# dremovd/PPO

Measured on AMD Instinct MI355X. Metric: env-steps/sec (Pong-shaped synthetic, 256 envs/GPU), higher is better.
Workload: dtype f32

## Files before the change

ppo_amd/csrc/stack_fused.hip:

```cpp
#include <cstdlib>
#include <type_traits>

#include "common.h"
#include "conv_stage.h"
#include "mfma.h"

#ifndef PPO_TAIL_SPLIT
#define PPO_TAIL_SPLIT 2
#endif

namespace ppo {
namespace {

constexpr int kScrPitchS = 20;

struct StackTailArgs {
    const float *in;
    const float *w[4];
    const float *bias[4];
    const float *mask[4];
    float *save[4];
    int n_images;
};

// ... 141 lines not shown
                    if (s < KS) {
#pragma unroll
                        for (int m = 0; m < MT; ++m)
#pragma unroll
                            for (int n = 0; n < NT; ++n) acc[n][m] = mfma16(wa[n][s], bv[u][m], acc[n][m]);
                    }
                }
                __builtin_amdgcn_sched_barrier(0);
            }

            __builtin_amdgcn_sched_barrier(0);
            load_weights((layer + 1) & 3);
            float *dst = smem + (odd ? 0 : S::LDS_MAP);
            float *save = a.save[layer];
            __builtin_amdgcn_sched_barrier(0);
            float skip[MT][NT][4];
#pragma unroll
            for (int m = 0; m < MT; ++m)
#pragma unroll
                for (int n = 0; n < NT; ++n)
#pragma unroll
                    for (int r = 0; r < 4; ++r)
                        skip[m][n][r] = odd ? smem[((n0 + n) * 16 + g * 4 + r) * PLANE + G + W + (pix[m] < S::NPIX ? pix[m] : 0)] : 0.f;
#pragma unroll
            for (int m = 0; m < MT; ++m) {
                if (pix[m] < S::NPIX) {
#pragma unroll
                    for (int n = 0; n < NT; ++n)
#pragma unroll
                        for (int r = 0; r < 4; ++r) {
                            const int co = (n0 + n) * 16 + g * 4 + r;
                            const int lo = co * PLANE + G + W + pix[m];
                            float val = acc[n][m][r] + bias_r[n][r];
                            if constexpr (BACKWARD) val = gate[m][n][r] > 0.f ? val : 0.f;
                            if (odd) val = val + skip[m][n][r];
                            dst[lo] = val;
                            if (save) save[img_off + (size_t)co * (H * W) + pix[m]] = val;
                        }
                }
            }
        }
    }
}

template <int C, int H, int W, int MT, int NW, int NSPLIT, bool BACKWARD>
int launch_stack_tail(const StackTailArgs &args, hipStream_t st)
{
    using S = StackCfg<C, H, W, MT, NW, NSPLIT>;
    constexpr auto kern = stack_tail_kernel<C, H, W, MT, NW, NSPLIT, BACKWARD>;
    int nb = 0;
    if (int rc = prepare_kernel<kern>("stack_tail", S::LDS_BYTES, S::WAVES * 64, &nb)) return rc;
    const int wg_per_cu = nb < 1 ? 1 : nb;
    int grid = 256 * wg_per_cu;
    if (grid > args.n_images) grid = args.n_images;
    hipLaunchKernelGGL(kern, dim3(grid), dim3(S::WAVES * 64), S::LDS_BYTES, st, args);
    return check_launch("stack_tail_kernel");
}

template <int C, int H, int W, int TR>
struct ShiftCfg {
    static_assert(C == 16, "one channel tile per wave");
    static constexpr int NW = 16;
    static constexpr int GW = 8;
    static constexpr int G = 4;
    static constexpr int PITCH = W + 2;
    static constexpr int ROWS = H + 6;
    static constexpr int PLANE_RAW = ROWS * PITCH + 2 * G;
    static constexpr int PLANE = PLANE_RAW + ((16 - PLANE_RAW % 32) + 32) % 32;
    static constexpr int KS = 9 * (C / 4);
    static constexpr int NBANDS = (H + TR - 1) / TR;
    static constexpr int NPIX = TR * W;
    static constexpr int MTILES = (NPIX + 15) / 16;
    static constexpr int MT = MTILES / GW;
    static constexpr int LDS_MAP = C * PLANE;
    static constexpr int SCR = MT * 16 * kScrPitchS;
    static constexpr size_t LDS_BYTES = (size_t)(LDS_MAP + GW * SCR) * 4;
    static_assert(H % TR == 0 && MTILES == MT * GW, "whole bands, tiles split evenly over a group's waves");
    static_assert((H * W) % 4 == 0 && NPIX % 4 == 0 && W % 2 == 0, "float4 epilogue on whole quads");
    static_assert(LDS_BYTES <= 160 * 1024, "map + scratch must fit the CU's LDS");
};

template <int C, int H, int W, int TR, bool BACKWARD>
__global__ __launch_bounds__(1024) void stack_shift_kernel(StackTailArgs a)
{
    using S = ShiftCfg<C, H, W, TR>;
    constexpr int KS = S::KS, PLANE = S::PLANE, PITCH = S::PITCH, G = S::G, MT = S::MT, NW = S::NW;
    extern __shared__ __align__(16) float smem[];
    const int tid = threadIdx.x, lane = tid & 63, l15 = lane & 15, g = lane >> 4, wave = tid >> 6;
    const int grp = __builtin_amdgcn_readfirstlane(wave / S::GW), wv = wave % S::GW;
    const int ch = lane >> 2, quad = lane & 3;
    float *scr = smem + S::LDS_MAP + wv * S::SCR;

    zero_lds<S::LDS_MAP, NW * 64>(smem, tid);

    int lofs[MT], p4[MT], po[MT][2];
#pragma unroll
    for (int m = 0; m < MT; ++m) {
        const int p = (wv * MT + m) * 16 + l15;
        lofs[m] = G + (p / W) * PITCH + p % W - 1 + g * PLANE;
        p4[m] = (wv * MT + m) * 16 + quad * 4;
        po[m][0] = (p4[m] / W) * PITCH + p4[m] % W;
        po[m][1] = ((p4[m] + 2) / W) * PITCH + (p4[m] + 2) % W;
    }

    for (int img = blockIdx.x; img < a.n_images; img += gridDim.x) {
        const size_t img_off = (size_t)img * C * H * W;
        __syncthreads();
        for (int i = tid; i < C * 6 * W; i += NW * 64) {
            const int c = i / (6 * W), r = (i / W) % 6, x = i % W;
            smem[c * PLANE + G + (r < 5 ? r : H + 5) * PITCH + x] = 0.f;
        }
        {
            constexpr int W2 = W / 2, RP = 64 / W2, NQ = H / RP;
            static_assert(H % RP == 0, "whole requests");
            const int w0 = __builtin_amdgcn_readfirstlane(wave);
            const bool live = lane < RP * W2;
            const int ls = live ? lane : RP * W2 - 1;
            for (int c = w0; c < C; c += NW) {
                const float2 *g2 = reinterpret_cast<const float2 *>(a.in + img_off + (size_t)c * H * W) + ls;
                float *l0 = smem + c * PLANE + G + (5 + ls / W2) * PITCH + (ls % W2) * 2;
                float2 v[NQ];
#pragma unroll
                for (int q = 0; q < NQ; ++q) v[q] = g2[q * RP * W2];
#pragma unroll
                for (int q = 0; q < NQ; ++q) {
                    const float2 o = BACKWARD ? v[q] : make_float2(relu1(v[q].x), relu1(v[q].y));
                    if (live) *reinterpret_cast<float2 *>(l0 + q * RP * PITCH) = o;
                }
            }
        }

#pragma unroll 1
        for (int layer = 0; layer < 4; ++layer) {
            float wa[KS];
            const float4 *pw = reinterpret_cast<const float4 *>(a.w[layer]);
#pragma unroll
            for (int s4 = 0; s4 < KS / 4; ++s4) {
                const float4 v = pw[s4 * 64 + lane];
                wa[4 * s4 + 0] = v.x, wa[4 * s4 + 1] = v.y, wa[4 * s4 + 2] = v.z, wa[4 * s4 + 3] = v.w;
            }
            const float bias_c = BACKWARD ? 0.f : a.bias[layer][ch];
            const int odd = layer & 1;
            const float *res = odd ? (layer == 1 ? a.in : a.save[1]) + img_off : nullptr;
            const float *mask = BACKWARD ? a.mask[layer] + img_off : nullptr;
            float *save = a.save[layer] ? a.save[layer] + img_off : nullptr;
            const __amdgpu_buffer_rsrc_t mask_b = buffer_of(mask, mask != nullptr), res_b = buffer_of(res, res != nullptr);
            const int in_row = 5 - layer;

            f32x4 acc[MT];
            float4 gate4[MT], res4[MT];

            __syncthreads();
#pragma unroll 1
            for (int hs = 0; hs <= S::NBANDS; ++hs) {
                if ((hs & 1) == grp) {
                    if (hs < S::NBANDS) {
                        const int y0 = hs * TR;
                        const int chan_off = ch * (H * W) + y0 * W;
#pragma unroll
                        for (int m = 0; m < MT; ++m) {
                            const bool live = p4[m] < S::NPIX;
                            const int off = live ? (chan_off + p4[m]) * 4 : kOutside;
                            if constexpr (BACKWARD) gate4[m] = buffer_f32x4(mask_b, off);
                            res4[m] = buffer_f32x4(res_b, off);
                        }
                        constexpr int CS_HI = ((C / 4 - 1) * 4 * PLANE + 2 * PITCH + 2) * 4 > 65535 ? C / 8 : C / 4;
                        static_assert(((C / 4 - 1 - (CS_HI < C / 4 ? CS_HI : 0)) * 4 * PLANE + 2 * PITCH + 2) * 4 <= 65535 &&
                                      ((CS_HI - 1) * 4 * PLANE + 2 * PITCH + 2) * 4 <= 65535, "operand offsets fit the instruction");
                        using lds_cvf = const volatile __attribute__((address_space(3))) float;
                        lds_cvf *vsmem = (lds_cvf *)smem;
                        int base[MT], base_hi[MT];
#pragma unroll
                        for (int m = 0; m < MT; ++m) {
                            base[m] = lofs[m] + (y0 - 1 + in_row) * PITCH;
                            base_hi[m] = base[m] + CS_HI * 4 * PLANE;
                            if constexpr (CS_HI < C / 4) asm volatile("" : "+v"(base_hi[m]));
                            acc[m] = f32x4{0.f, 0.f, 0.f, 0.f};
                        }
                        constexpr int SB = 2;
                        constexpr int NB = (KS + SB - 1) / SB;
                        float raw[2][SB][MT];
                        auto load_block = [&](int j, float (&r)[SB][MT]) {
#pragma unroll
                            for (int u = 0; u < SB; ++u) {
                                const int s = j * SB + u;
                                if (s < KS) {
                                    const int tap = s / (C / 4), cs = s % (C / 4);
                                    const int tap_off = (tap / 3) * PITCH + (tap % 3);
#pragma unroll
                                    for (int m = 0; m < MT; ++m)
                                        r[u][m] = cs < CS_HI ? vsmem[base[m] + cs * 4 * PLANE + tap_off]
                                                             : vsmem[base_hi[m] + (cs - CS_HI) * 4 * PLANE + tap_off];
                                }
                            }
                        };
                        load_block(0, raw[0]);
#pragma unroll
                        for (int j = 0; j < NB; ++j) {
                            __builtin_amdgcn_sched_barrier(0);
                            if (j + 1 < NB) load_block(j + 1, raw[(j + 1) & 1]);
                            __builtin_amdgcn_sched_barrier(0);
#pragma unroll
                            for (int u = 0; u < SB; ++u) {
                                const int s = j * SB + u;
                                if (s < KS) {
#pragma unroll
                                    for (int m = 0; m < MT; ++m) acc[m] = mfma16(wa[s], raw[j & 1][u][m], acc[m]);
                                }
                            }
                            __builtin_amdgcn_sched_barrier(0);
                        }
                    } else if (layer < 3) {
                        for (int i = tid % (S::GW * 64); i < C * W; i += S::GW * 64)
                            smem[(i / W) * PLANE + G + (H + in_row - 1) * PITCH + i % W] = 0.f;
                    }
                } else if (hs >= 1) {
                    const int y0 = (hs - 1) * TR;
                    const int chan_off = ch * (H * W) + y0 * W;
#pragma unroll
                    for (int m = 0; m < MT; ++m)
#pragma unroll
                        for (int r = 0; r < 4; ++r) scr[(m * 16 + g * 4 + r) * kScrPitchS + l15] = acc[m][r];
                    __builtin_amdgcn_wave_barrier();
                    float *out_row = smem + ch * PLANE + G + (y0 + in_row - 1) * PITCH;
#pragma unroll
                    for (int m = 0; m < MT; ++m) {
                        if (p4[m] >= S::NPIX) continue;
                        const float4 o = *reinterpret_cast<const float4 *>(scr + (m * 16 + ch) * kScrPitchS + quad * 4);
                        const float ov[4] = {o.x, o.y, o.z, o.w};
                        const float gv[4] = {gate4[m].x, gate4[m].y, gate4[m].z, gate4[m].w};
                        const float rv[4] = {res4[m].x, res4[m].y, res4[m].z, res4[m].w};
                        float v[4];
#pragma unroll
                        for (int e = 0; e < 4; ++e) {
                            float val = ov[e] + bias_c;
                            if constexpr (BACKWARD) val = gv[e] > 0.f ? val : 0.f;
                            v[e] = val + rv[e];
                        }
                        if (layer < 3) {
                            float t[4];
#pragma unroll
                            for (int e = 0; e < 4; ++e) t[e] = BACKWARD ? v[e] : relu1(v[e]);
                            *reinterpret_cast<float2 *>(out_row + po[m][0]) = make_float2(t[0], t[1]);
                            *reinterpret_cast<float2 *>(out_row + po[m][1]) = make_float2(t[2], t[3]);
                        }
                        if (save) *reinterpret_cast<float4 *>(save + chan_off + p4[m]) = make_float4(v[0], v[1], v[2], v[3]);
                    }
                    __builtin_amdgcn_wave_barrier();
                }
                __syncthreads();
            }
        }
    }
}

template <int C, int H, int W, int TR, bool BACKWARD>
int launch_stack_shift(const StackTailArgs &args, hipStream_t st)
{
    using S = ShiftCfg<C, H, W, TR>;
    constexpr auto kern = stack_shift_kernel<C, H, W, TR, BACKWARD>;
    if (int rc = prepare_kernel<kern>("stack_shift", S::LDS_BYTES)) return rc;
    int grid = 256;
    if (grid > args.n_images) grid = args.n_images;
    hipLaunchKernelGGL(kern, dim3(grid), dim3(S::NW * 64), S::LDS_BYTES, st, args);
    return check_launch("stack_shift_kernel");
}

template <int I, int N, class F>
__device__ __forceinline__ void static_for(F &&f)
{
    if constexpr (I < N) {
        f(std::integral_constant<int, I>{});
        static_for<I + 1, N>(f);
    }
}

struct LaneMap {
    template <int MT>
    struct T {
        int pix[MT], lofs[MT];
        float hi_l[MT], hi_r[MT];
    };
};

template <int H, int W, int PLANE, int G, int MT, int PITCH = W>
__device__ __forceinline__ void lane_map_init(LaneMap::T<MT> &lm, int pixel_wave, int l15, int g)
{
#pragma unroll
    for (int m = 0; m < MT; ++m) {
        const int p = (pixel_wave * MT + m) * 16 + l15;
        lm.pix[m] = p;
        const int pc = p < H * W ? p : 0;
        if constexpr (PITCH == W) {
            lm.lofs[m] = G + pc - 1 + g * PLANE;
            lm.hi_l[m] = (pc % W == 0) ? 0.f : INFINITY;
            lm.hi_r[m] = (pc % W == W - 1) ? 0.f : INFINITY;
        } else {
            lm.lofs[m] = G + (pc / W) * PITCH + pc % W - 1 + g * PLANE;
            lm.hi_l[m] = lm.hi_r[m] = 0.f;
        }
    }
}

template <int C, int H, int W, int MT, int NTOT, int NT, bool RELU_IN, bool GATED = false, int PITCH = W>
__device__ __forceinline__ void resident_conv(float *smem, int src_off, int dst_off, bool residual, const float *wpk,
                                              const float *bias, float *save, const LaneMap::T<MT> &lm, int n0, int lane,
                                              const float *mask = nullptr)
{
    constexpr int ROWS = H + 2, G = 4, PLANE_RAW = ROWS * PITCH + 2 * G;
    constexpr int PLANE = PLANE_RAW + ((16 - PLANE_RAW % 32) + 32) % 32;
    constexpr int KS = 9 * (C / 4);
    constexpr bool PADDED = PITCH != W;
    static_assert(!PADDED || (PITCH == W + 1 && !RELU_IN), "padded maps hold what the MFMA takes: identity input only");
    const int g = lane >> 4;
    float wa[NT][KS];
    const float4 *pw = reinterpret_cast<const float4 *>(wpk);
#pragma unroll
    for (int s4 = 0; s4 < KS / 4; ++s4)
#pragma unroll
        for (int n = 0; n < NT; ++n) {
            const float4 v = pw[(s4 * NTOT + n0 + n) * 64 + lane];
            wa[n][4 * s4 + 0] = v.x;
            wa[n][4 * s4 + 1] = v.y;
            wa[n][4 * s4 + 2] = v.z;
            wa[n][4 * s4 + 3] = v.w;
        }
    float bias_r[NT][4];
#pragma unroll
    for (int n = 0; n < NT; ++n)
#pragma unroll
        for (int r = 0; r < 4; ++r) bias_r[n][r] = (GATED || !bias) ? 0.f : bias[(n0 + n) * 16 + g * 4 + r];
    constexpr int SB = (MT * NT >= 4) ? 2 : 4;
    constexpr int NB = (KS + SB - 1) / SB;
    constexpr int GATE_AT = (GATED && MT * NT * 4 > 16) ? NB / 2 : -1;
    float gate[GATED ? MT : 1][NT][4];
    auto load_gate = [&]() {
        const __amdgpu_buffer_rsrc_t mask_b = buffer_of(mask);
#pragma unroll
        for (int m = 0; m < MT; ++m)
#pragma unroll
            for (int n = 0; n < NT; ++n)
#pragma unroll
                for (int r = 0; r < 4; ++r)
                    gate[m][n][r] = buffer_f32(mask_b, lm.pix[m] < H * W ? (((n0 + n) * 16 + g * 4 + r) * (H * W) + lm.pix[m]) * 4
                                                                         : kOutside);
    };
    if constexpr (GATED && GATE_AT < 0) load_gate();

    __syncthreads();
    int base[MT];
#pragma unroll
    for (int m = 0; m < MT; ++m) {
        base[m] = lm.lofs[m] + src_off;
        if constexpr (PADDED) asm volatile("" : "+v"(base[m]));
    }
    f32x4 acc[NT][MT];
#pragma unroll
    for (int n = 0; n < NT; ++n)
#pragma unroll
        for (int m = 0; m < MT; ++m) acc[n][m] = f32x4{0.f, 0.f, 0.f, 0.f};

    float raw[2][SB][MT];
    auto load_block = [&](int j, float (&r)[SB][MT]) {
#pragma unroll
        for (int u = 0; u < SB; ++u) {
            const int s = j * SB + u;
            if (s < KS) {
                const int tap = s / (C / 4), cs = s % (C / 4);
                const int tap_off = (tap / 3) * PITCH + (tap % 3);
#pragma unroll
                for (int m = 0; m < MT; ++m) {
                    if constexpr (PADDED) {
                        using lds_cvf = const volatile __attribute__((address_space(3))) float;
                        r[u][m] = ((lds_cvf *)smem)[base[m] + cs * 4 * PLANE + tap_off];
                    } else {
                        r[u][m] = smem[base[m] + cs * 4 * PLANE + tap_off];
                    }
                }
            }
        }
    };
    static_assert(!PADDED || ((C / 4 - 1) * 4 * PLANE + 2 * PITCH + 2) * 4 <= 65535, "operand offsets fit the instruction");
    load_block(0, raw[0]);
    static_for<0, NB>([&](auto jc) {
        constexpr int j = decltype(jc)::value;
        float bv[SB][MT];
#pragma unroll
        for (int u = 0; u < SB; ++u) {
            const int s = j * SB + u;
            if (s < KS) {
                const int kx = (s / (C / 4)) % 3;
#pragma unroll
                for (int m = 0; m < MT; ++m) {
                    float x = raw[j & 1][u][m];
                    if constexpr (PADDED) {
                    } else if (kx != 1) {
                        const float hi = kx == 0 ? lm.hi_l[m] : lm.hi_r[m];
                        x = __builtin_amdgcn_fmed3f(x, RELU_IN ? 0.f : -hi, hi);
                    } else if (RELU_IN) {
                        x = relu1(x);
                    }
                    bv[u][m] = x;
                }
            }
        }
        __builtin_amdgcn_sched_barrier(0);
        if constexpr (j + 1 < NB) load_block(j + 1, raw[(j + 1) & 1]);
        if constexpr (PADDED) __builtin_amdgcn_sched_barrier(0);
        if constexpr (j == GATE_AT) load_gate();
#pragma unroll
        for (int u = 0; u < SB; ++u) {
            const int s = j * SB + u;
            if (s < KS) {
#pragma unroll
                for (int m = 0; m < MT; ++m)
#pragma unroll
                    for (int n = 0; n < NT; ++n) acc[n][m] = mfma16(wa[n][s], bv[u][m], acc[n][m]);
            }
        }
        __builtin_amdgcn_sched_barrier(0);
    });
#pragma unroll
    for (int m = 0; m < MT; ++m) {
        if (lm.pix[m] < H * W) {
#pragma unroll
            for (int n = 0; n < NT; ++n)
#pragma unroll
                for (int r = 0; r < 4; ++r) {
                    const int co = (n0 + n) * 16 + g * 4 + r;
                    const int lo = PADDED ? dst_off + co * PLANE + (lm.lofs[m] - g * PLANE) + PITCH + 1
                                          : dst_off + co * PLANE + G + W + lm.pix[m];
                    float val = acc[n][m][r] + bias_r[n][r];
                    if constexpr (GATED) val = gate[m][n][r] > 0.f ? val : 0.f;
                    if (residual) val = val + smem[lo];
                    smem[lo] = val;
                    if (save) save[(size_t)co * (H * W) + lm.pix[m]] = val;
                }
        }
    }
}

struct StackFullArgs {
    const float *in;
    const float *w[5];
    const float *bias[5];
    float *pooled;
    uint8_t *argmax;
    float *save[4];
    const float *pre_w[4];
    const float *pre_bias[4];
    float *pre_save[4];
    int has_pre;
    int n_images;
};

template <int C, int HI, int WI, int MTI, int HO, int WO, int MTO, int NW, int NSPLIT>
__global__ __launch_bounds__(NW * NSPLIT * 64) void stack_full_kernel(StackFullArgs a)
{
    using SI = StackCfg<C, HI, WI, MTI, NW, NSPLIT>;
    using SO = StackCfg<C, HO, WO, MTO, NW, NSPLIT>;
    static_assert(HO == (HI + 1) / 2 && WO == (WI + 1) / 2, "3x3 / stride 2 / pad 1 pooling");
    static_assert(2 * SO::LDS_MAP <= SI::LDS_MAP, "the small maps reuse the input map's LDS");
    constexpr int NT = SI::NTL, WAVES = SI::WAVES, THREADS = WAVES * 64;
    constexpr int A_OFF = 0, B_OFF = SI::LDS_MAP, X_OFF = 0, Y_OFF = SO::LDS_MAP;
    extern __shared__ __align__(16) float smem[];
    const int tid = threadIdx.x, lane = tid & 63, l15 = lane & 15, g = lane >> 4;
    const int wave = tid >> 6, pixel_wave = wave % NW, n0 = (wave / NW) * NT;

    LaneMap::T<MTI> lmi;
    LaneMap::T<MTO> lmo;
    lane_map_init<HI, WI, SI::PLANE, SI::G, MTI>(lmi, pixel_wave, l15, g);
    lane_map_init<HO, WO, SO::PLANE, SO::G, MTO>(lmo, pixel_wave, l15, g);

    if (a.has_pre) zero_lds<SI::LDS_MAP, THREADS>(smem + B_OFF, tid);

    for (int img = blockIdx.x; img < a.n_images; img += gridDim.x) {
        __syncthreads();
        zero_lds<SI::LDS_MAP, THREADS>(smem + A_OFF, tid);
        __syncthreads();
        stage_band_chunk_dma<C, HI, WI, SI::ROWS, SI::PLANE, SI::G, WAVES>(a.in, img, 0, smem + A_OFF, tid);
        if (a.has_pre) {
            const size_t big_img = (size_t)img * C * HI * WI;
#pragma unroll 1
            for (int layer = 0; layer < 4; ++layer) {
                const int odd = layer & 1;
                float *save = a.pre_save[layer] ? a.pre_save[layer] + big_img : nullptr;
                resident_conv<C, HI, WI, MTI, SI::NT, NT, true>(smem, odd ? B_OFF : A_OFF, odd ? A_OFF : B_OFF, odd != 0,
                                                                a.pre_w[layer], a.pre_bias[layer], save, lmi, n0, lane);
            }
        }
        resident_conv<C, HI, WI, MTI, SI::NT, NT, false>(smem, A_OFF, B_OFF, false, a.w[0], a.bias[0], nullptr, lmi, n0, lane);
        __syncthreads();
        zero_lds<2 * SO::LDS_MAP, THREADS>(smem + X_OFF, tid);
        __syncthreads();
        {
            constexpr int RPW = 64 / WO;
            const int sub = lane / WO, xo = lane % WO;
            const size_t out_img = (size_t)img * C * HO * WO;
            for (int u0 = wave * RPW; u0 < C * HO; u0 += WAVES * RPW) {
                const int u = u0 + sub;
                const int co = u / HO, yo = u % HO;
                if (sub < RPW && co < C) {
                    const float *src = smem + B_OFF + co * SI::PLANE + SI::G + WI + (2 * yo - 1) * WI + 2 * xo - 1;
                    float best;
                    int best_tap;
                    pool_window_lds<HI % 2 == 0, WI % 2 == 0>(src, WI, yo > 0, 2 * yo + 1 < HI, xo > 0, 2 * xo + 1 < WI, best, best_tap);
                    smem[X_OFF + co * SO::PLANE + SO::G + WO + yo * WO + xo] = best;
                    const size_t oi = out_img + ((size_t)co * HO + yo) * WO + xo;
                    if (a.pooled) a.pooled[oi] = best;
                    if (a.argmax) a.argmax[oi] = (uint8_t)best_tap;
                }
            }
        }
        const size_t out_img = (size_t)img * C * HO * WO;
#pragma unroll 1
        for (int layer = 0; layer < 4; ++layer) {
            const int odd = layer & 1;
            float *save = a.save[layer] ? a.save[layer] + out_img : nullptr;
            resident_conv<C, HO, WO, MTO, SO::NT, NT, true>(smem, odd ? Y_OFF : X_OFF, odd ? X_OFF : Y_OFF, odd != 0,
                                                            a.w[1 + layer], a.bias[1 + layer], save, lmo, n0, lane);
        }
    }
}

struct StackFullBwdArgs {
    const float *g;
    const float *w[5];
    const float *mask[4];
    const uint8_t *argmax;
    float *save[4];
    float *dc;
    float *g_prev;
    const float *post_w[4];
    const float *post_mask[4];
    float *post_save[4];
    int has_post;
    int n_images;
};

template <int C, int HI, int WI, int MTI, int HO, int WO, int MTO, int NW, int NSPLIT>
__global__ __launch_bounds__(NW * NSPLIT * 64) void stack_full_bwd_kernel(StackFullBwdArgs a)
{
    using SI = StackCfg<C, HI, WI, MTI, NW, NSPLIT, WI + 1>;
    using SO = StackCfg<C, HO, WO, MTO, NW, NSPLIT, WO + 1>;
    static_assert(2 * SO::LDS_MAP <= SI::LDS_MAP, "the small maps live inside the first big map's LDS");
    static_assert(C * HO * WO <= SO::LDS_MAP * 4, "the argmax bytes of an image fit the second small map");
    constexpr int NT = SI::NTL, WAVES = SI::WAVES, THREADS = WAVES * 64;
    constexpr int A_OFF = 0, B_OFF = SI::LDS_MAP, X_OFF = 0, Y_OFF = SO::LDS_MAP;
    extern __shared__ __align__(16) float smem[];
    const int tid = threadIdx.x, lane = tid & 63, l15 = lane & 15, g = lane >> 4;
    const int wave = tid >> 6, pixel_wave = wave % NW, n0 = (wave / NW) * NT;

    LaneMap::T<MTI> lmi;
    LaneMap::T<MTO> lmo;
    lane_map_init<HI, WI, SI::PLANE, SI::G, MTI, SI::PITCH>(lmi, pixel_wave, l15, g);
    lane_map_init<HO, WO, SO::PLANE, SO::G, MTO, SO::PITCH>(lmo, pixel_wave, l15, g);

    zero_lds<SI::LDS_MAP, THREADS>(smem + B_OFF, tid);

    for (int img = blockIdx.x; img < a.n_images; img += gridDim.x) {
        __syncthreads();
        zero_lds<2 * SO::LDS_MAP, THREADS>(smem + X_OFF, tid);
        __syncthreads();
        const size_t small_img = (size_t)img * C * HO * WO, big_img = (size_t)img * C * HI * WI;
        for (int row = tid; row < C * HO; row += THREADS) {
            const float *gr = a.g + small_img + row * WO;
            float *lr = smem + X_OFF + (row / HO) * SO::PLANE + SO::G + (1 + row % HO) * SO::PITCH;
            float gv[WO];
#pragma unroll
            for (int x = 0; x < WO; ++x) gv[x] = gr[x];
#pragma unroll
            for (int x = 0; x < WO; ++x) lr[x] = gv[x];
        }
        constexpr int AM_WORDS = C * HO * WO / 4, AM_PER = (AM_WORDS + THREADS - 1) / THREADS;
        static_assert(C * HO * WO % 4 == 0, "an image's argmax bytes are whole words (the entry points check the base)");
        uint32_t am_r[AM_PER];
#pragma unroll
        for (int k = 0; k < AM_PER; ++k) {
            const int i = tid + k * THREADS;
            am_r[k] = reinterpret_cast<const uint32_t *>(a.argmax + small_img)[i < AM_WORDS ? i : 0];
        }
#pragma unroll 1
        for (int layer = 0; layer < 4; ++layer) {
            const int odd = layer & 1;
            resident_conv<C, HO, WO, MTO, SO::NT, NT, false, true, SO::PITCH>(smem, odd ? Y_OFF : X_OFF, odd ? X_OFF : Y_OFF, odd != 0,
                                                                   a.w[layer], nullptr, a.save[layer] + small_img, lmo, n0,
                                                                   lane, a.mask[layer] + small_img);
        }
        __syncthreads();
        const uint8_t *am = reinterpret_cast<const uint8_t *>(smem + Y_OFF);
#pragma unroll
        for (int k = 0; k < AM_PER; ++k) {
            const int i = tid + k * THREADS;
            if (i < AM_WORDS) reinterpret_cast<uint32_t *>(smem + Y_OFF)[i] = am_r[k];
        }
        __syncthreads();
        {
            for (int e = tid; e < C * HI * WI; e += THREADS) {
                const int co = e / (HI * WI), r = e % (HI * WI);
                const int iy = r / WI, ix = r % WI;
                const int k = ix >> 1, oy0 = iy >> 1;
                const int ky0 = (iy & 1) ? 2 : 1;
                const bool has_oy1 = (iy & 1) && (oy0 + 1 < HO);
                const bool odd_x = ix & 1;
                const bool has_ox1 = odd_x && (k + 1 < WO);
                const int kx0 = odd_x ? 2 : 1;
                const float *gx = smem + X_OFF + co * SO::PLANE + SO::G + SO::PITCH;
                const uint8_t *ac = am + co * (HO * WO);
                float sum = 0.f;
                {
                    const int i00 = oy0 * WO + k, x00 = oy0 * SO::PITCH + k;
                    if (ac[i00] == ky0 * 3 + kx0) sum += gx[x00];
                    if (has_ox1 && ac[i00 + 1] == ky0 * 3 + 0) sum += gx[x00 + 1];
                }
                if (has_oy1) {
                    const int i10 = (oy0 + 1) * WO + k, x10 = (oy0 + 1) * SO::PITCH + k;
                    if (ac[i10] == kx0) sum += gx[x10];
                    if (has_ox1 && ac[i10 + 1] == 0) sum += gx[x10 + 1];
                }
                smem[B_OFF + co * SI::PLANE + SI::G + (1 + iy) * SI::PITCH + ix] = sum;
                a.dc[big_img + e] = sum;
            }
        }
        if (a.has_post) {
            __syncthreads();
            zero_lds<SI::LDS_MAP, THREADS>(smem + A_OFF, tid);
        }
        resident_conv<C, HI, WI, MTI, SI::NT, NT, false, false, SI::PITCH>(smem, B_OFF, A_OFF, false, a.w[4], nullptr,
                                                                a.g_prev + big_img, lmi, n0, lane);
        if (a.has_post) {
#pragma unroll 1
            for (int layer = 0; layer < 4; ++layer) {
                const int odd = layer & 1;
                resident_conv<C, HI, WI, MTI, SI::NT, NT, false, true, SI::PITCH>(smem, odd ? B_OFF : A_OFF, odd ? A_OFF : B_OFF, odd != 0,
                                                                       a.post_w[layer], nullptr, a.post_save[layer] + big_img,
                                                                       lmi, n0, lane, a.post_mask[layer] + big_img);
            }
        }
    }
}

template <int C, int HI, int WI, int MTI, int HO, int WO, int MTO, int NW, int NSPLIT>
int launch_stack_full(const StackFullBwdArgs &args, hipStream_t st)
{
    using SI = StackCfg<C, HI, WI, MTI, NW, NSPLIT, WI + 1>;
    constexpr size_t kLds = 2 * (size_t)SI::LDS_MAP * 4;
    static_assert(kLds <= 160 * 1024, "two padded maps fit the CU's LDS");
    constexpr auto kern = stack_full_bwd_kernel<C, HI, WI, MTI, HO, WO, MTO, NW, NSPLIT>;
    if (int rc = prepare_kernel<kern>("stack_full_bwd", kLds)) return rc;
    const int grid = args.n_images < 256 ? args.n_images : 256;
    hipLaunchKernelGGL(kern, dim3(grid), dim3(SI::WAVES * 64), kLds, st, args);
    return check_launch("stack_full_bwd_kernel");
}

template <int C, int HI, int WI, int MTI, int HO, int WO, int MTO, int NW, int NSPLIT>
int launch_stack_full(const StackFullArgs &args, hipStream_t st)
{
    using SI = StackCfg<C, HI, WI, MTI, NW, NSPLIT>;
    constexpr size_t kLds = 2 * (size_t)SI::LDS_MAP * 4;
    constexpr auto kern = stack_full_kernel<C, HI, WI, MTI, HO, WO, MTO, NW, NSPLIT>;
    if (int rc = prepare_kernel<kern>("stack_full", kLds)) return rc;
    const int grid = args.n_images < 256 ? args.n_images : 256;
    hipLaunchKernelGGL(kern, dim3(grid), dim3(SI::WAVES * 64), kLds, st, args);
    return check_launch("stack_full_kernel");
}


struct ChainSplitArgs {
    const float *in;
    const float *pre_w[4];
    const float *pre_bias[4];
    const float *w[5];
    const float *bias[5];
    float *out;
    float *xbuf;
    uint32_t *flags;
    uint32_t *ctl;
    int n_images;
    int skip;
};

constexpr int kSplitWaves = 8;
constexpr uint32_t kSpinLimit = 1u << 21;

template <int C, int HI, int WI, int HO, int WO>
__global__ __launch_bounds__(kSplitWaves * 64) void stack_chain_split_kernel(ChainSplitArgs a)
{
    static_assert(C == 32, "two channel tiles: one per workgroup of a pair");
    using SI = StackCfg<C, HI, WI, 7, 4, 2>;
    using SO = StackCfg<C, HO, WO, 2, 4, 2>;
    constexpr int MTI = 4, MTO = 2, WAVES = kSplitWaves, THREADS = WAVES * 64;
    static_assert(SI::MTILES <= MTI * WAVES && SO::MTILES == MTO * 4 && WAVES == 8, "every pixel tile has a wave");
    static_assert(2 * SO::LDS_MAP <= SI::LDS_MAP, "the small maps reuse the input map's LDS");
    constexpr int A_OFF = 0, B_OFF = SI::LDS_MAP, X_OFF = 0, Y_OFF = SO::LDS_MAP;
    extern __shared__ __align__(16) float smem[];
    const int tid = threadIdx.x, lane = tid & 63, l15 = lane & 15, g = lane >> 4;
    const int wave = tid >> 6;
    const int b = blockIdx.x;
    const int h = (b >> 3) & 1;
    const int pair0 = (b & 7) | ((b >> 4) << 3);
    const int n_pairs = (gridDim.x >> 4) << 3;

    LaneMap::T<MTI> lmi;
    LaneMap::T<MTO> lmo;
    lane_map_init<HI, WI, SI::PLANE, SI::G, MTI>(lmi, wave, l15, g);
    lane_map_init<HO, WO, SO::PLANE, SO::G, MTO>(lmo, wave & 3, l15, g);

    const uint32_t base = __hip_atomic_load(a.ctl, __ATOMIC_RELAXED, __HIP_MEMORY_SCOPE_AGENT) * 8u;
    const uint32_t fault = __hip_atomic_load(a.ctl + 3, __ATOMIC_RELAXED, __HIP_MEMORY_SCOPE_AGENT);
    const uint32_t spin_limit = fault ? 1u << 10 : kSpinLimit;
    bool gave_up = false;
    zero_lds<SI::LDS_MAP, THREADS>(smem + B_OFF, tid);

    for (int img = pair0; img < a.n_images; img += n_pairs) {
        uint32_t *flag_own = a.flags + 2 * img + h, *flag_other = a.flags + 2 * img + (1 - h);
        float *slots = a.xbuf + (size_t)img * 2 * C * HI * WI;
        uint32_t step = 0;
        auto exchange = [&](int dst_off, float *slot, bool fetch) {
            ++step;
            asm volatile("s_waitcnt vmcnt(0)" ::: "memory");
            __syncthreads();
            if (tid == 0) {
                if (!(fault && h == 1))
                    __hip_atomic_store(flag_own, base + step, __ATOMIC_RELAXED, __HIP_MEMORY_SCOPE_AGENT);
                uint32_t it = 0;
                while (!(a.skip & 1) && !gave_up &&
                       __hip_atomic_load(flag_other, __ATOMIC_RELAXED, __HIP_MEMORY_SCOPE_AGENT) < base + step) {
                    if (++it > spin_limit ||
                        ((it & 1023u) == 0 && __hip_atomic_load(a.ctl + 2, __ATOMIC_RELAXED, __HIP_MEMORY_SCOPE_AGENT))) {
                        __hip_atomic_store(a.ctl + 2, 1u, __ATOMIC_RELAXED, __HIP_MEMORY_SCOPE_AGENT);
                        gave_up = true;
                        break;
                    }
                    __builtin_amdgcn_s_sleep(2);
                }
            }
            __syncthreads();
            if (fetch)
                stage_band_chunk_dma<16, HI, WI, SI::ROWS, SI::PLANE, SI::G, WAVES, 16>(slot + (size_t)(1 - h) * 16 * HI * WI, 0, 0,
                                                                                       smem + dst_off + (1 - h) * 16 * SI::PLANE, tid);
        };

        __syncthreads();
        zero_lds<SI::LDS_MAP, THREADS>(smem + A_OFF, tid);
        __syncthreads();
        stage_band_chunk_dma<C, HI, WI, SI::ROWS, SI::PLANE, SI::G, WAVES>(a.in, img, 0, smem + A_OFF, tid);
#pragma unroll 1
        for (int layer = 0; layer < 4; ++layer) {
            const int odd = layer & 1;
            float *slot = slots + (size_t)(layer & 1) * C * HI * WI;
            resident_conv<C, HI, WI, MTI, 2, 1, true>(smem, odd ? B_OFF : A_OFF, odd ? A_OFF : B_OFF, odd != 0, a.pre_w[layer],
                                                      a.pre_bias[layer], slot, lmi, h, lane);
            exchange(odd ? A_OFF : B_OFF, slot, true);
        }
        resident_conv<C, HI, WI, MTI, 2, 1, false>(smem, A_OFF, B_OFF, false, a.w[0], a.bias[0], slots, lmi, h, lane);
        exchange(B_OFF, slots, h == 0);
        if (h != 0 || (a.skip & 2)) continue;
        __syncthreads();
        zero_lds<2 * SO::LDS_MAP, THREADS>(smem + X_OFF, tid);
        __syncthreads();
        {
            constexpr int RPW = 64 / WO;
            const int sub = lane / WO, xo = lane % WO;
            for (int u0 = wave * RPW; u0 < C * HO; u0 += WAVES * RPW) {
                const int u = u0 + sub;
                const int co = u / HO, yo = u % HO;
                if (sub < RPW && co < C) {
                    const float *src = smem + B_OFF + co * SI::PLANE + SI::G + WI + (2 * yo - 1) * WI + 2 * xo - 1;
                    float best;
                    int best_tap;
                    pool_window_lds<HI % 2 == 0, WI % 2 == 0>(src, WI, yo > 0, 2 * yo + 1 < HI, xo > 0, 2 * xo + 1 < WI, best, best_tap);
                    smem[X_OFF + co * SO::PLANE + SO::G + WO + yo * WO + xo] = best;
                }
            }
        }
        float *out_img = a.out + (size_t)img * C * HO * WO;
#pragma unroll 1
        for (int layer = 0; layer < 4; ++layer) {
            const int odd = layer & 1;
            resident_conv<C, HO, WO, MTO, 2, 1, true>(smem, odd ? Y_OFF : X_OFF, odd ? X_OFF : Y_OFF, odd != 0, a.w[1 + layer],
                                                      a.bias[1 + layer], layer == 3 ? out_img : nullptr, lmo, wave >> 2, lane);
        }
    }
    __syncthreads();
    if (tid == 0) {
        const uint32_t done = __hip_atomic_fetch_add(a.ctl + 1, 1u, __ATOMIC_RELAXED, __HIP_MEMORY_SCOPE_AGENT);
        if (done == gridDim.x - 1) {
            __hip_atomic_store(a.ctl + 1, 0u, __ATOMIC_RELAXED, __HIP_MEMORY_SCOPE_AGENT);
            __hip_atomic_fetch_add(a.ctl, 1u, __ATOMIC_RELAXED, __HIP_MEMORY_SCOPE_AGENT);
        }
    }
}

template <int C, int HI, int WI, int HO, int WO>
int launch_chain_split(const ChainSplitArgs &args, hipStream_t st)
{
    using SI = StackCfg<C, HI, WI, 7, 4, 2>;
    constexpr size_t kLds = 2 * (size_t)SI::LDS_MAP * 4;
    constexpr auto kern = stack_chain_split_kernel<C, HI, WI, HO, WO>;
    if (int rc = prepare_kernel<kern>("stack_chain_split", kLds)) return rc;
    int groups = (args.n_images + 7) / 8;
    if (groups > 16) groups = 16;
    hipLaunchKernelGGL(kern, dim3(16 * groups), dim3(kSplitWaves * 64), kLds, st, args);
    return check_launch("stack_chain_split_kernel");
}

#define PPO_STACK_CASE(LAUNCH, C, H, W, ...) \
    if (channels == C && h == H && w == W) return args ? LAUNCH<C, H, W, __VA_ARGS__>(*args, st) : PPO_OK;

int no_kernel(const char *who, int channels, int h, int w)
{
    return fail(PPO_E_INVALID, "%s: no kernel for %d channels at %dx%d", who, channels, h, w);
}

template <bool BACKWARD>
int dispatch_stack_tail(const char *who, int channels, int h, int w, const StackTailArgs *args, hipStream_t st)
{
    PPO_STACK_CASE(launch_stack_shift, 16, 42, 42, 6, BACKWARD)
    PPO_STACK_CASE(launch_stack_shift, 16, 32, 32, 8, BACKWARD)
    PPO_STACK_CASE(launch_stack_tail, 32, 11, 11, 2, 4, PPO_TAIL_SPLIT, BACKWARD)
    PPO_STACK_CASE(launch_stack_tail, 32, 21, 21, 7, 4, PPO_TAIL_SPLIT, BACKWARD)
    PPO_STACK_CASE(launch_stack_tail, 32, 16, 16, 4, 4, PPO_TAIL_SPLIT, BACKWARD)
    PPO_STACK_CASE(launch_stack_tail, 32, 8, 8, 1, 4, PPO_TAIL_SPLIT, BACKWARD)
    return args ? no_kernel(who, channels, h, w) : PPO_E_INVALID;
}

template <class Args>
int dispatch_stack_full(const char *who, int channels, int h, int w, const Args *args, hipStream_t st)
{
    PPO_STACK_CASE(launch_stack_full, 32, 21, 21, 7, 11, 11, 2, 4, 2)
    PPO_STACK_CASE(launch_stack_full, 32, 16, 16, 4, 8, 8, 1, 4, 2)
    return args ? no_kernel(who, channels, h, w) : PPO_E_INVALID;
}

int dispatch_chain_split(const char *who, int channels, int h, int w, const ChainSplitArgs *args, hipStream_t st)
{
    PPO_STACK_CASE(launch_chain_split, 32, 21, 21, 11, 11)
    return args ? no_kernel(who, channels, h, w) : PPO_E_INVALID;
}
#undef PPO_STACK_CASE

template <int N, int M>
int fill_layers(const char *who, const char *other, const float *const *weights, const float *const *others,
                const float *(&w)[N], const float *(&o)[M])
{
    for (int l = 0; l < N; ++l) {
        if (!weights[l] || (l < M && !others[l])) return fail(PPO_E_INVALID, "%s: null weights / %s of layer %d", who, other, l);
        if (!aligned(weights[l], 16)) return fail(PPO_E_ALIGN, "%s: packed weights must be 16-byte aligned", who);
        w[l] = weights[l];
        if (l < M) o[l] = others[l];
    }
    return PPO_OK;
}

struct ChainedStack {
    const float *const *weights, *const *others;
    float *save[4];
};

int stack_full_forward(const char *who, const float *in, const ChainedStack *pre, const float *const *packed_weights,
                       const float *const *biases, float *pooled, uint8_t *argmax, float *a0, float *q0, float *a1, float *q1,
                       int n_images, int channels, int h, int w, void *stream)
{
    if (n_images < 0) return fail(PPO_E_INVALID, "%s: negative batch", who);
    if (n_images == 0) return PPO_OK;
    if (!in || !packed_weights || !biases || !q1 || (pre && (!pre->weights || !pre->others)))
        return fail(PPO_E_INVALID, "%s: null pointer", who);
    StackFullArgs args{};
    args.in = in, args.pooled = pooled, args.argmax = argmax, args.n_images = n_images;
    args.save[0] = a0, args.save[1] = q0, args.save[2] = a1, args.save[3] = q1;
    if (int rc = fill_layers(who, "bias", packed_weights, biases, args.w, args.bias)) return rc;
    if (pre) {
        if (int rc = fill_layers(who, "bias", pre->weights, pre->others, args.pre_w, args.pre_bias)) return rc;
        for (int l = 0; l < 4; ++l) args.pre_save[l] = pre->save[l];
        args.has_pre = 1;
    }
    return dispatch_stack_full(who, channels, h, w, &args, as_stream(stream));
}

int stack_full_backward(const char *who, const float *g, const float *const *packed_weights_t, const float *const *masks,
                        const uint8_t *argmax, float *da1, float *g1, float *da0, float *g0, float *dc, float *g_prev,
                        const ChainedStack *post, int n_images, int channels, int h, int w, void *stream)
{
    if (n_images < 0) return fail(PPO_E_INVALID, "%s: negative batch", who);
    if (n_images == 0) return PPO_OK;
    if (!g || !packed_weights_t || !masks || !argmax || !da1 || !g1 || !da0 || !g0 || !dc || !g_prev ||
        (post && (!post->weights || !post->others || !post->save[0] || !post->save[1] || !post->save[2] || !post->save[3])))
        return fail(PPO_E_INVALID, "%s: null pointer", who);
    if (!aligned(argmax, 4)) return fail(PPO_E_ALIGN, "%s: argmax must be 4-byte aligned", who);
    StackFullBwdArgs args{};
    args.g = g, args.argmax = argmax, args.dc = dc, args.g_prev = g_prev, args.n_images = n_images;
    args.save[0] = da1, args.save[1] = g1, args.save[2] = da0, args.save[3] = g0;
    if (int rc = fill_layers(who, "mask", packed_weights_t, masks, args.w, args.mask)) return rc;
    if (post) {
        if (int rc = fill_layers(who, "mask", post->weights, post->others, args.post_w, args.post_mask)) return rc;
        for (int l = 0; l < 4; ++l) args.post_save[l] = post->save[l];
        args.has_post = 1;
    }
    return dispatch_stack_full(who, channels, h, w, &args, as_stream(stream));
}

struct ChainSplitLayout {
    size_t flags, ctl, bytes;
};
ChainSplitLayout chain_split_layout(int n_images, int channels, int h, int w)
{
    const size_t slots = (size_t)n_images * 2 * channels * h * w * sizeof(float);
    const size_t flags = ((size_t)n_images * 2 * sizeof(uint32_t) + 15) & ~(size_t)15;
    return {slots, slots + flags, slots + flags + 16};
}

}
}

extern "C" int ppo_impala_stack_tail_supported(int channels, int h, int w)
{
    return ppo::dispatch_stack_tail<false>(nullptr, channels, h, w, nullptr, nullptr) == PPO_OK;
}

extern "C" int ppo_impala_stack_tail_forward_f32(const float *in, const float *const *packed_weights,
                                                 const float *const *biases, float *a0, float *q0, float *a1, float *q1,
                                                 int n_images, int channels, int h, int w, void *stream)
{
    using namespace ppo;
    const char *who = "ppo_impala_stack_tail_forward_f32";
    if (n_images < 0) return fail(PPO_E_INVALID, "%s: negative batch", who);
    if (n_images == 0) return PPO_OK;
    if (!in || !packed_weights || !biases || !q1) return fail(PPO_E_INVALID, "%s: null pointer", who);
    StackTailArgs args{};
    args.in = in, args.n_images = n_images;
    args.save[0] = a0, args.save[1] = q0, args.save[2] = a1, args.save[3] = q1;
    if (int rc = fill_layers(who, "bias", packed_weights, biases, args.w, args.bias)) return rc;
    if (!aligned(in, 4)) return fail(PPO_E_ALIGN, "%s: input must be 4-byte aligned", who);
    if (channels == 16) {
        if (!q0) return fail(PPO_E_INVALID, "%s: the 16-channel form needs q0 (its second block re-reads it)", who);
        if (!aligned(in, 16) || !aligned(q0, 16) || !aligned(q1, 16) || (a0 && !aligned(a0, 16)) || (a1 && !aligned(a1, 16)))
            return fail(PPO_E_ALIGN, "%s: the 16-channel form needs 16-byte aligned maps", who);
    }
    return dispatch_stack_tail<false>(who, channels, h, w, &args, as_stream(stream));
}

extern "C" int ppo_impala_stack_tail_backward_f32(const float *g, const float *const *packed_weights_t,
                                                  const float *const *masks, float *da1, float *g1, float *da0, float *g0,
                                                  int n_images, int channels, int h, int w, void *stream)
{
    using namespace ppo;
    const char *who = "ppo_impala_stack_tail_backward_f32";
    if (n_images < 0) return fail(PPO_E_INVALID, "%s: negative batch", who);
    if (n_images == 0) return PPO_OK;
    if (!g || !packed_weights_t || !masks || !da1 || !g1 || !da0 || !g0) return fail(PPO_E_INVALID, "%s: null pointer", who);
    StackTailArgs args{};
    args.in = g, args.n_images = n_images;
    args.save[0] = da1, args.save[1] = g1, args.save[2] = da0, args.save[3] = g0;
    if (int rc = fill_layers(who, "mask", packed_weights_t, masks, args.w, args.mask)) return rc;
    if (channels == 16)
        for (const void *ptr : {(const void *)g, (const void *)da1, (const void *)g1, (const void *)da0, (const void *)g0,
                                (const void *)masks[0], (const void *)masks[1], (const void *)masks[2], (const void *)masks[3]})
            if (!aligned(ptr, 16)) return fail(PPO_E_ALIGN, "%s: the 16-channel form needs 16-byte aligned maps", who);
    return dispatch_stack_tail<true>(who, channels, h, w, &args, as_stream(stream));
}

extern "C" int ppo_impala_stack_full_supported(int channels, int h, int w)
{
    return ppo::dispatch_stack_full<ppo::StackFullArgs>(nullptr, channels, h, w, nullptr, nullptr) == PPO_OK;
}

extern "C" int ppo_impala_stack_full_forward_f32(const float *in, const float *const *packed_weights,
                                                 const float *const *biases, float *pooled, uint8_t *argmax, float *a0,
                                                 float *q0, float *a1, float *q1, int n_images, int channels, int h, int w,
                                                 void *stream)
{
    return ppo::stack_full_forward("ppo_impala_stack_full_forward_f32", in, nullptr, packed_weights, biases, pooled, argmax, a0,
                                   q0, a1, q1, n_images, channels, h, w, stream);
}

extern "C" int ppo_impala_stack_chain_forward_f32(const float *in, const float *const *pre_packed_weights,
                                                  const float *const *pre_biases, float *pre_a0, float *pre_q0,
                                                  float *pre_a1, float *pre_q1, const float *const *packed_weights,
                                                  const float *const *biases, float *pooled, uint8_t *argmax, float *a0,
                                                  float *q0, float *a1, float *q1, int n_images, int channels, int h, int w,
                                                  void *stream)
{
    const ppo::ChainedStack pre{pre_packed_weights, pre_biases, {pre_a0, pre_q0, pre_a1, pre_q1}};
    return ppo::stack_full_forward("ppo_impala_stack_chain_forward_f32", in, &pre, packed_weights, biases, pooled, argmax, a0,
                                   q0, a1, q1, n_images, channels, h, w, stream);
}

extern "C" int ppo_impala_stack_full_backward_f32(const float *g, const float *const *packed_weights_t,
                                                  const float *const *masks, const uint8_t *argmax, float *da1, float *g1,
                                                  float *da0, float *g0, float *dc, float *g_prev, int n_images,
                                                  int channels, int h, int w, void *stream)
{
    return ppo::stack_full_backward("ppo_impala_stack_full_backward_f32", g, packed_weights_t, masks, argmax, da1, g1, da0, g0,
                                    dc, g_prev, nullptr, n_images, channels, h, w, stream);
}

extern "C" int ppo_impala_stack_chain_backward_f32(const float *g, const float *const *packed_weights_t,
                                                   const float *const *masks, const uint8_t *argmax, float *da1, float *g1,
                                                   float *da0, float *g0, float *dc, float *g_prev,
                                                   const float *const *post_packed_weights_t, const float *const *post_masks,
                                                   float *post_da1, float *post_g1, float *post_da0, float *post_g0,
                                                   int n_images, int channels, int h, int w, void *stream)
{
    const ppo::ChainedStack post{post_packed_weights_t, post_masks, {post_da1, post_g1, post_da0, post_g0}};
    return ppo::stack_full_backward("ppo_impala_stack_chain_backward_f32", g, packed_weights_t, masks, argmax, da1, g1, da0, g0,
                                    dc, g_prev, &post, n_images, channels, h, w, stream);
}

extern "C" size_t ppo_impala_stack_chain_split_workspace_bytes(int n_images, int channels, int h, int w)
{
    return ppo::chain_split_layout(n_images, channels, h, w).bytes;
}

extern "C" int ppo_impala_stack_chain_split_forward_f32(const float *in, const float *const *pre_packed_weights,
                                                        const float *const *pre_biases,
                                                        const float *const *packed_weights, const float *const *biases,
                                                        float *q1, void *workspace, size_t workspace_bytes, int n_images,
                                                        int channels, int h, int w, void *stream)
{
    using namespace ppo;
    const char *who = "ppo_impala_stack_chain_split_forward_f32";
    if (n_images < 0) return fail(PPO_E_INVALID, "%s: negative batch", who);
    if (n_images == 0) return PPO_OK;
    if (!in || !pre_packed_weights || !pre_biases || !packed_weights || !biases || !q1 || !workspace)
        return fail(PPO_E_INVALID, "%s: null pointer", who);
    if (dispatch_chain_split(who, channels, h, w, nullptr, nullptr) != PPO_OK) return no_kernel(who, channels, h, w);
    const ChainSplitLayout at = chain_split_layout(n_images, channels, h, w);
    if (workspace_bytes < at.bytes || !aligned(workspace, 16)) return fail(PPO_E_INVALID, "%s: workspace too small or misaligned", who);
    ChainSplitArgs args{};
    args.in = in, args.out = q1, args.n_images = n_images;
    if (int rc = fill_layers(who, "bias", packed_weights, biases, args.w, args.bias)) return rc;
    if (int rc = fill_layers(who, "bias", pre_packed_weights, pre_biases, args.pre_w, args.pre_bias)) return rc;
    args.xbuf = static_cast<float *>(workspace);
    args.flags = reinterpret_cast<uint32_t *>(static_cast<char *>(workspace) + at.flags);
    args.ctl = reinterpret_cast<uint32_t *>(static_cast<char *>(workspace) + at.ctl);
#ifdef PPO_TUNE_TIMING_AIDS
    static const int skip = getenv("PPO_AMD_SPLIT_SKIP") ? atoi(getenv("PPO_AMD_SPLIT_SKIP")) : 0;
    args.skip = skip;
#endif
    return dispatch_chain_split(who, channels, h, w, &args, as_stream(stream));
}
```

Before: 101,300.

## Prefetch next layer's conv weights into registers and batch residual LDS reads

Each resident conv used to load its own A-operand weights from global memory at entry. Now a single register array is kept across layers, and the next layer's weights are loaded right after the MFMA loop, so that global load latency overlaps the epilogue. For maps other than 16 high, the residual values are also read from LDS in one batch before the stores instead of interleaved with them. The cost is more live registers and possible occupancy loss, plus careful selection of which weight comes next across branches.

```diff
diff --git a/ppo_amd/csrc/stack_fused.hip b/ppo_amd/csrc/stack_fused.hip
--- a/ppo_amd/csrc/stack_fused.hip
+++ b/ppo_amd/csrc/stack_fused.hip
@@ -467,8 +467,34 @@
     }
 }
 
-template <int C, int H, int W, int MT, int NTOT, int NT, bool RELU_IN, bool GATED = false, int PITCH = W>
-__device__ __forceinline__ void resident_conv(float *smem, int src_off, int dst_off, bool residual, const float *wpk,
+#ifndef PPO_TUNE_RESIDENT_PREFETCH
+#define PPO_TUNE_RESIDENT_PREFETCH 1
+#endif
+constexpr bool kResidentPrefetch = PPO_TUNE_RESIDENT_PREFETCH != 0;
+constexpr bool resident_batched_skip(int hi) { return kResidentPrefetch && hi != 16; }
+
+template <int NTOT, int NT, int KS>
+__device__ __forceinline__ void load_a_operand(float (&wa)[NT][KS], const float *wpk, int n0, int lane)
+{
+    const float4 *pw = reinterpret_cast<const float4 *>(wpk);
+    int at = n0 * 64 + lane;
+    asm volatile("" : "+v"(at));
+#pragma unroll
+    for (int s4 = 0; s4 < KS / 4; ++s4)
+#pragma unroll
+        for (int n = 0; n < NT; ++n) {
+            const float4 v = pw[(s4 * NTOT + n) * 64 + at];
+            wa[n][4 * s4 + 0] = v.x;
+            wa[n][4 * s4 + 1] = v.y;
+            wa[n][4 * s4 + 2] = v.z;
+            wa[n][4 * s4 + 3] = v.w;
+        }
+}
+
+template <int C, int H, int W, int MT, int NTOT, int NT, bool RELU_IN, bool GATED = false, int PITCH = W,
+          bool PREFETCH = false, bool BATCH_SKIP = PREFETCH>
+__device__ __forceinline__ void resident_conv(float *smem, int src_off, int dst_off, bool residual,
+                                              float (&wa)[NT][9 * (C / 4)], const float *wpk, const float *next_w, int next_n0,
                                               const float *bias, float *save, const LaneMap::T<MT> &lm, int n0, int lane,
                                               const float *mask = nullptr)
 {
@@ -478,18 +504,7 @@
     constexpr bool PADDED = PITCH != W;
     static_assert(!PADDED || (PITCH == W + 1 && !RELU_IN), "padded maps hold what the MFMA takes: identity input only");
     const int g = lane >> 4;
-    float wa[NT][KS];
-    const float4 *pw = reinterpret_cast<const float4 *>(wpk);
-#pragma unroll
-    for (int s4 = 0; s4 < KS / 4; ++s4)
-#pragma unroll
-        for (int n = 0; n < NT; ++n) {
-            const float4 v = pw[(s4 * NTOT + n0 + n) * 64 + lane];
-            wa[n][4 * s4 + 0] = v.x;
-            wa[n][4 * s4 + 1] = v.y;
-            wa[n][4 * s4 + 2] = v.z;
-            wa[n][4 * s4 + 3] = v.w;
-        }
+    if constexpr (!PREFETCH) load_a_operand<NTOT>(wa, wpk, n0, lane);
     float bias_r[NT][4];
 #pragma unroll
     for (int n = 0; n < NT; ++n)
@@ -585,6 +600,25 @@
         }
         __builtin_amdgcn_sched_barrier(0);
     });
+    auto place = [&](int m, int n, int r) {
+        const int co = (n0 + n) * 16 + g * 4 + r;
+        return PADDED ? dst_off + co * PLANE + (lm.lofs[m] - g * PLANE) + PITCH + 1
+                      : dst_off + co * PLANE + G + W + (lm.pix[m] < H * W ? lm.pix[m] : 0);
+    };
+    float skip[BATCH_SKIP ? MT : 1][NT][4];
+    if constexpr (PREFETCH) {
+        __builtin_amdgcn_sched_barrier(0);
+        load_a_operand<NTOT>(wa, next_w, next_n0, lane);
+        __builtin_amdgcn_sched_barrier(0);
+    }
+    if constexpr (BATCH_SKIP) {
+#pragma unroll
+        for (int m = 0; m < MT; ++m)
+#pragma unroll
+            for (int n = 0; n < NT; ++n)
+#pragma unroll
+                for (int r = 0; r < 4; ++r) skip[m][n][r] = residual ? smem[place(m, n, r)] : 0.f;
+    }
 #pragma unroll
     for (int m = 0; m < MT; ++m) {
         if (lm.pix[m] < H * W) {
@@ -593,11 +627,14 @@
 #pragma unroll
                 for (int r = 0; r < 4; ++r) {
                     const int co = (n0 + n) * 16 + g * 4 + r;
-                    const int lo = PADDED ? dst_off + co * PLANE + (lm.lofs[m] - g * PLANE) + PITCH + 1
-                                          : dst_off + co * PLANE + G + W + lm.pix[m];
+                    const int lo = place(m, n, r);
                     float val = acc[n][m][r] + bias_r[n][r];
                     if constexpr (GATED) val = gate[m][n][r] > 0.f ? val : 0.f;
-                    if (residual) val = val + smem[lo];
+                    if constexpr (BATCH_SKIP) {
+                        if (residual) val = val + skip[m][n][r];
+                    } else {
+                        if (residual) val = val + smem[lo];
+                    }
                     smem[lo] = val;
                     if (save) save[(size_t)co * (H * W) + lm.pix[m]] = val;
                 }
@@ -627,6 +664,7 @@
     static_assert(HO == (HI + 1) / 2 && WO == (WI + 1) / 2, "3x3 / stride 2 / pad 1 pooling");
     static_assert(2 * SO::LDS_MAP <= SI::LDS_MAP, "the small maps reuse the input map's LDS");
     constexpr int NT = SI::NTL, WAVES = SI::WAVES, THREADS = WAVES * 64;
+    constexpr bool PF = kResidentPrefetch, BS = resident_batched_skip(HI);
     constexpr int A_OFF = 0, B_OFF = SI::LDS_MAP, X_OFF = 0, Y_OFF = SO::LDS_MAP;
     extern __shared__ __align__(16) float smem[];
     const int tid = threadIdx.x, lane = tid & 63, l15 = lane & 15, g = lane >> 4;
@@ -638,6 +676,10 @@
     lane_map_init<HO, WO, SO::PLANE, SO::G, MTO>(lmo, pixel_wave, l15, g);
 
     if (a.has_pre) zero_lds<SI::LDS_MAP, THREADS>(smem + B_OFF, tid);
+
+    float wa[NT][SI::KS];
+    const float *first_w = a.has_pre ? a.pre_w[0] : a.w[0];
+    if constexpr (PF) load_a_operand<SI::NT>(wa, first_w, n0, lane);
 
     for (int img = blockIdx.x; img < a.n_images; img += gridDim.x) {
         __syncthreads();
@@ -650,11 +692,13 @@
             for (int layer = 0; layer < 4; ++layer) {
                 const int odd = layer & 1;
                 float *save = a.pre_save[layer] ? a.pre_save[layer] + big_img : nullptr;
-                resident_conv<C, HI, WI, MTI, SI::NT, NT, true>(smem, odd ? B_OFF : A_OFF, odd ? A_OFF : B_OFF, odd != 0,
-                                                                a.pre_w[layer], a.pre_bias[layer], save, lmi, n0, lane);
-            }
-        }
-        resident_conv<C, HI, WI, MTI, SI::NT, NT, false>(smem, A_OFF, B_OFF, false, a.w[0], a.bias[0], nullptr, lmi, n0, lane);
+                resident_conv<C, HI, WI, MTI, SI::NT, NT, true, false, WI, PF, BS>(smem, odd ? B_OFF : A_OFF, odd ? A_OFF : B_OFF, odd != 0, wa,
+                                                                a.pre_w[layer], layer < 3 ? a.pre_w[layer + 1] : a.w[0], n0,
+                                                                a.pre_bias[layer], save, lmi, n0, lane);
+            }
+        }
+        resident_conv<C, HI, WI, MTI, SI::NT, NT, false, false, WI, PF, BS>(smem, A_OFF, B_OFF, false, wa, a.w[0], a.w[1], n0, a.bias[0],
+                                                                        nullptr, lmi, n0, lane);
         __syncthreads();
         zero_lds<2 * SO::LDS_MAP, THREADS>(smem + X_OFF, tid);
         __syncthreads();
@@ -682,8 +726,9 @@
         for (int layer = 0; layer < 4; ++layer) {
             const int odd = layer & 1;
             float *save = a.save[layer] ? a.save[layer] + out_img : nullptr;
-            resident_conv<C, HO, WO, MTO, SO::NT, NT, true>(smem, odd ? Y_OFF : X_OFF, odd ? X_OFF : Y_OFF, odd != 0,
-                                                            a.w[1 + layer], a.bias[1 + layer], save, lmo, n0, lane);
+            resident_conv<C, HO, WO, MTO, SO::NT, NT, true, false, WO, PF, BS>(smem, odd ? Y_OFF : X_OFF, odd ? X_OFF : Y_OFF, odd != 0, wa,
+                                                            a.w[1 + layer], layer < 3 ? a.w[2 + layer] : first_w, n0,
+                                                            a.bias[1 + layer], save, lmo, n0, lane);
         }
     }
 }
@@ -711,6 +756,7 @@
     static_assert(2 * SO::LDS_MAP <= SI::LDS_MAP, "the small maps live inside the first big map's LDS");
     static_assert(C * HO * WO <= SO::LDS_MAP * 4, "the argmax bytes of an image fit the second small map");
     constexpr int NT = SI::NTL, WAVES = SI::WAVES, THREADS = WAVES * 64;
+    constexpr bool PF = kResidentPrefetch, BS = resident_batched_skip(HI);
     constexpr int A_OFF = 0, B_OFF = SI::LDS_MAP, X_OFF = 0, Y_OFF = SO::LDS_MAP;
     extern __shared__ __align__(16) float smem[];
     const int tid = threadIdx.x, lane = tid & 63, l15 = lane & 15, g = lane >> 4;
@@ -722,6 +768,9 @@
     lane_map_init<HO, WO, SO::PLANE, SO::G, MTO, SO::PITCH>(lmo, pixel_wave, l15, g);
 
     zero_lds<SI::LDS_MAP, THREADS>(smem + B_OFF, tid);
+
+    float wa[NT][SI::KS];
+    if constexpr (PF) load_a_operand<SI::NT>(wa, a.w[0], n0, lane);
 
     for (int img = blockIdx.x; img < a.n_images; img += gridDim.x) {
         __syncthreads();
@@ -748,9 +797,10 @@
 #pragma unroll 1
         for (int layer = 0; layer < 4; ++layer) {
             const int odd = layer & 1;
-            resident_conv<C, HO, WO, MTO, SO::NT, NT, false, true, SO::PITCH>(smem, odd ? Y_OFF : X_OFF, odd ? X_OFF : Y_OFF, odd != 0,
-                                                                   a.w[layer], nullptr, a.save[layer] + small_img, lmo, n0,
-                                                                   lane, a.mask[layer] + small_img);
+            resident_conv<C, HO, WO, MTO, SO::NT, NT, false, true, SO::PITCH, PF, BS>(smem, odd ? Y_OFF : X_OFF, odd ? X_OFF : Y_OFF,
+                                                                       odd != 0, wa, a.w[layer], a.w[layer + 1], n0, nullptr,
+                                                                       a.save[layer] + small_img, lmo, n0, lane,
+                                                                       a.mask[layer] + small_img);
         }
         __syncthreads();
         const uint8_t *am = reinterpret_cast<const uint8_t *>(smem + Y_OFF);
@@ -791,15 +841,18 @@
             __syncthreads();
             zero_lds<SI::LDS_MAP, THREADS>(smem + A_OFF, tid);
         }
-        resident_conv<C, HI, WI, MTI, SI::NT, NT, false, false, SI::PITCH>(smem, B_OFF, A_OFF, false, a.w[4], nullptr,
-                                                                a.g_prev + big_img, lmi, n0, lane);
+        resident_conv<C, HI, WI, MTI, SI::NT, NT, false, false, SI::PITCH, PF, BS>(smem, B_OFF, A_OFF, false, wa, a.w[4],
+                                                                    a.has_post ? a.post_w[0] : a.w[0], n0, nullptr,
+                                                                    a.g_prev + big_img, lmi, n0, lane);
         if (a.has_post) {
 #pragma unroll 1
             for (int layer = 0; layer < 4; ++layer) {
                 const int odd = layer & 1;
-                resident_conv<C, HI, WI, MTI, SI::NT, NT, false, true, SI::PITCH>(smem, odd ? B_OFF : A_OFF, odd ? A_OFF : B_OFF, odd != 0,
-                                                                       a.post_w[layer], nullptr, a.post_save[layer] + big_img,
-                                                                       lmi, n0, lane, a.post_mask[layer] + big_img);
+                resident_conv<C, HI, WI, MTI, SI::NT, NT, false, true, SI::PITCH, PF, BS>(smem, odd ? B_OFF : A_OFF, odd ? A_OFF : B_OFF,
+                                                                           odd != 0, wa, a.post_w[layer],
+                                                                           layer < 3 ? a.post_w[layer + 1] : a.w[0], n0, nullptr,
+                                                                           a.post_save[layer] + big_img, lmi, n0, lane,
+                                                                           a.post_mask[layer] + big_img);
             }
         }
     }
@@ -876,6 +929,10 @@
     const uint32_t spin_limit = fault ? 1u << 10 : kSpinLimit;
     bool gave_up = false;
     zero_lds<SI::LDS_MAP, THREADS>(smem + B_OFF, tid);
+
+    float wa[1][SI::KS];
+    constexpr bool PF = kResidentPrefetch, BS = resident_batched_skip(HI);
+    if constexpr (PF) load_a_operand<2>(wa, a.pre_w[0], h, lane);
 
     for (int img = pair0; img < a.n_images; img += n_pairs) {
         uint32_t *flag_own = a.flags + 2 * img + h, *flag_other = a.flags + 2 * img + (1 - h);
@@ -914,13 +971,16 @@
         for (int layer = 0; layer < 4; ++layer) {
             const int odd = layer & 1;
             float *slot = slots + (size_t)(layer & 1) * C * HI * WI;
-            resident_conv<C, HI, WI, MTI, 2, 1, true>(smem, odd ? B_OFF : A_OFF, odd ? A_OFF : B_OFF, odd != 0, a.pre_w[layer],
-                                                      a.pre_bias[layer], slot, lmi, h, lane);
+            resident_conv<C, HI, WI, MTI, 2, 1, true, false, WI, PF, BS>(smem, odd ? B_OFF : A_OFF, odd ? A_OFF : B_OFF, odd != 0, wa, a.pre_w[layer],
+                                                      layer < 3 ? a.pre_w[layer + 1] : a.w[0], h, a.pre_bias[layer], slot, lmi,
+                                                      h, lane);
             exchange(odd ? A_OFF : B_OFF, slot, true);
         }
-        resident_conv<C, HI, WI, MTI, 2, 1, false>(smem, A_OFF, B_OFF, false, a.w[0], a.bias[0], slots, lmi, h, lane);
+        const bool leaves = h != 0 || (a.skip & 2);
+        resident_conv<C, HI, WI, MTI, 2, 1, false, false, WI, PF, BS>(smem, A_OFF, B_OFF, false, wa, a.w[0], leaves ? a.pre_w[0] : a.w[1],
+                                                   leaves ? h : wave >> 2, a.bias[0], slots, lmi, h, lane);
         exchange(B_OFF, slots, h == 0);
-        if (h != 0 || (a.skip & 2)) continue;
+        if (leaves) continue;
         __syncthreads();
         zero_lds<2 * SO::LDS_MAP, THREADS>(smem + X_OFF, tid);
         __syncthreads();
@@ -943,7 +1003,8 @@
 #pragma unroll 1
         for (int layer = 0; layer < 4; ++layer) {
             const int odd = layer & 1;
-            resident_conv<C, HO, WO, MTO, 2, 1, true>(smem, odd ? Y_OFF : X_OFF, odd ? X_OFF : Y_OFF, odd != 0, a.w[1 + layer],
+            resident_conv<C, HO, WO, MTO, 2, 1, true, false, WO, PF, BS>(smem, odd ? Y_OFF : X_OFF, odd ? X_OFF : Y_OFF, odd != 0, wa, a.w[1 + layer],
+                                                      layer < 3 ? a.w[2 + layer] : a.pre_w[0], layer < 3 ? wave >> 2 : h,
                                                       a.bias[1 + layer], layer == 3 ? out_img : nullptr, lmo, wave >> 2, lane);
         }
     }
```

Result: no change. 102,000, median of 6 (+0.7%).
